# ArmingLou/seed-vc

Measured on AMD Instinct MI355X. Metric: mel_frames_per_sec, higher is better.
Workload: dtype f16; 1 GPU; seed-uvit-tat-xlsr-tiny CFM 25 steps cfg 0.7 + HiFT, batch 64 x (P=430,S=430) per GPU; batch_per_gpu=64, global_batch=64, prompt_frames=430, diffusion_steps=25, vocoder_precision=fp16p8, lanes_per_gpu=2, parallelism=utterance-sharded x1, audio gather on rank 0

## Files before the change

### seed-vc_amd/csrc/common.h

```cpp
#pragma once
#include <atomic>
#include <hip/hip_runtime.h>
#include <stdint.h>
#include <stdio.h>
#include <string>

namespace svc {

typedef _Float16 half_t;
typedef _Float16 half8 __attribute__((ext_vector_type(8)));
typedef _Float16 half4 __attribute__((ext_vector_type(4)));
typedef _Float16 half2v __attribute__((ext_vector_type(2)));
typedef float float4v __attribute__((ext_vector_type(4)));
typedef unsigned int u32x4 __attribute__((ext_vector_type(4)));

void set_error(const std::string& msg);
const char* get_error();

#define SVC_CHECK_HIP(expr)                                                                  \
    do {                                                                                     \
        hipError_t _e = (expr);                                                              \
        if (_e != hipSuccess) {                                                              \
            svc::set_error(std::string(#expr) + ": " + hipGetErrorString(_e) + " at " + __FILE__ + \
                           ":" + std::to_string(__LINE__));                                  \
            return 1;                                                                        \
        }                                                                                    \
    } while (0)

#define SVC_REQUIRE(cond, msg)                                                               \
    do {                                                                                     \
        if (!(cond)) {                                                                       \
            svc::set_error(std::string("requirement failed: ") + #cond + " -- " + (msg));    \
            return 1;                                                                        \
        }                                                                                    \
    } while (0)

__device__ __forceinline__ float sin_sq(float x) {
    const float n = rintf(x * 0.318309886183790672f);
    float r = fmaf(n, -3.140625f, x);
    r = fmaf(n, -9.67502593994140625e-4f, r);
    r = fmaf(n, -1.509957990978376e-7f, r);
    const float r2 = r * r;
    float p = fmaf(r2, 2.6348154733568663e-06f, -0.00019822761532850564f);
    p = fmaf(p, r2, 0.008333242498338223f);
    p = fmaf(p, r2, -0.1666666567325592f);
    const float sn = fmaf(p * r2, r, r);
    return sn * sn;
}

struct DeviceState {
    int device = -1;
    void* zero_page = nullptr;
    std::atomic<unsigned long long> kconv_attr{0};
    std::atomic<bool> fused_attr{false};
};
DeviceState* device_state();
int current_device();

enum { PROF_KGEMM_F16 = 0, PROF_KGEMM_F32 = 1, PROF_ATTN = 2, PROF_FUSED = 3, PROF_N = 4 };
bool prof_enabled();
void prof_begin(int cls, hipStream_t st);
void prof_end(int cls, double flops, double bytes, hipStream_t st, unsigned long long tag = 0);

template <int MAXA, int DPT>
__device__ __forceinline__ void wait_tiles(int ahead) {
    static_assert(MAXA * DPT <= 63, "vmcnt is a 6-bit counter");
    if constexpr (MAXA <= 0) {
        asm volatile("s_waitcnt vmcnt(0)" ::: "memory");
    } else {
        if (ahead >= MAXA) asm volatile("s_waitcnt vmcnt(%0)" ::"n"(MAXA * DPT) : "memory");
        else wait_tiles<MAXA - 1, DPT>(ahead);
    }
}

__device__ __forceinline__ float act_apply(float v, int act, float slope);
__device__ __forceinline__ uint4 pack8(const float* v) {
    half8 h;
#pragma unroll
    for (int j = 0; j < 8; ++j) h[j] = (half_t)v[j];
    return *reinterpret_cast<uint4*>(&h);
}

static inline int cdiv(long a, long b) { return (int)((a + b - 1) / b); }
static inline long round_up(long a, long b) { return (a + b - 1) / b * b; }

constexpr int KG_MAX_TAPS = 48;

enum { KG_PAD_ZERO = 0, KG_PAD_REFLECT = 1, KG_PAD_CLAMP = 2 };
enum { KG_ACT_NONE = 0, KG_ACT_SILU = 1, KG_ACT_ELU = 2, KG_ACT_LRELU = 3, KG_ACT_TANH = 4, KG_ACT_ABS = 5,
       KG_ACT_CLAMP = 6 , KG_ACT_SIGMOID = 7 };
enum {
    KG_EPI_STORE = 0,
    KG_EPI_SWIGLU = 1,
    KG_EPI_TANHSIG = 2,
    KG_EPI_QKV_ROPE = 3,
};

__device__ __forceinline__ float act_apply(float v, int act, float slope) {
    switch (act) {
        case KG_ACT_SILU: return v / (1.0f + __expf(-v));
        case KG_ACT_ELU: return v > 0.f ? v : (expm1f(v));
        case KG_ACT_LRELU: return v > 0.f ? v : v * slope;
        case KG_ACT_TANH: return tanhf(v);
        case KG_ACT_ABS: return fabsf(v);
        case KG_ACT_CLAMP: return fminf(fmaxf(v, -slope), slope);
        case KG_ACT_SIGMOID: return 1.0f / (1.0f + __expf(-v));
        default: return v;
// ... 44 lines not shown
    const void* w; long ldw;
    const float* bias;
    int B, Lin, Lout, N, cin_pad, k, dil, pad_left, nsub;
    int c_seq_rows, c_off;
    float* c32; long ldc32;
    half_t* c16; half_t* c16_lo; long ldc16;
    const float* post_a; const float* post_ib; int post_n;
    const float* res; long ldres;
    const float* res2; long ldres2;
    float out_scale;
    int act; float act_slope;
    const void* zero_page;
    int w8_exp;
    int c16_lo_fmt;
    const int* seq_len;
};
bool kconv_enabled();
int kconv_launch(const KConvParams& p, hipStream_t st);
__device__ __forceinline__ unsigned lo_pair_p8(float hi_as_float, float lo) {
    const float a = __builtin_amdgcn_fmed3f(hi_as_float, -448.f, 448.f), b = __builtin_amdgcn_fmed3f(lo * 2048.f, -448.f, 448.f);
    return (unsigned)__builtin_amdgcn_cvt_pk_fp8_f32(a, b, 0, false) & 0xffffu;
}
int kconv_pack_p8(const float* src, unsigned short* dst, int n0, int n1, int n2, long s0, long s1, long s2, long d0, long d1, long d2,
                  const float* scale, int* exp_out, hipStream_t st);

struct PanelParams {
    int M;
    int Lout, seq_rows, row_off;
    const half_t* wstream;
    int n_slots;
    float eps;
    int do_post;
    const half_t* ao;
    float* x;
    const float* gate_a; const float* gate_f;
    const float* g_ffn; const float* w_f; const float* b_f; int add_one;
    int I;
    half_t* c16;
    int do_skip;
    const half_t* skip_in; const float* bskip;
    int do_qkv;
    const float* g_attn; const float* w_a; const float* b_a;
    const float* rope; float q_scale;
    half_t* qk; half_t* vt; long vt_seq_stride; long vt_ld; int vt_mode;
    int do_final;
    const float* g_fin; const float* w_fin; const float* b_fin; half_t* n16;
};
bool fused_supported(int D, int I);
long fused_stream_halfs(int D, int I, bool post, bool skip, bool qkv);
long fused_pack_stream(half_t* dst, int D, int I, const float* wo, const float* w1, const float* w3, const float* w2,
                       const float* wskip, const float* wqkv, hipStream_t st);
int fused_panel_launch(const PanelParams& p, int D, bool gated, hipStream_t st);

struct AttnParams {
    const half_t* q; const half_t* k; long ld_qk;
    const half_t* vt; long vt_seq_stride; long vt_ld;
    half_t* out; long ld_out;
    int n_seq, H, seq_rows, Tq;
    int q_start;
    const int* kv_len; int kv_len_const;
    int vt_perm;
};
__host__ __device__ inline int vt_perm_pos(int pos) {
    return (pos & ~31) | (((pos >> 2) & 3) << 3) | (((pos >> 4) & 1) << 2) | (pos & 3);
}
__host__ __device__ inline int vt_perm_pos16(int pos) {
    return (pos & ~12) | ((pos & 4) << 1) | ((pos & 8) >> 1);
}
__host__ __device__ inline int vt_pos(int pos, int mode) {
    return mode == 2 ? vt_perm_pos16(pos) : (mode == 1 ? vt_perm_pos(pos) : pos);
}
int attention_vt_mode(int n_seq, int H, int Tq);
int attention_launch(const AttnParams& p, hipStream_t st);
int attention_permute_vt(half_t* vt, long rows, long vt_ld, int mode, hipStream_t st);

int rmsnorm_mod_launch(const float* x, long ldx, half_t* y, long ldy, const float* gamma,
                       const float* w, const float* b, long ld_wb, int add_one,
                       int rows, int D, int seq_rows, float eps, hipStream_t st);
int layernorm_mod_launch(const float* x, long ldx, half_t* y, long ldy, const float* scale,
                         const float* shift, int rows, int D, float eps, hipStream_t st);

}
```

### seed-vc_amd/csrc/dit.hip

```cpp
#include <math.h>
#include <string.h>

#include <algorithm>
#include <vector>

#include "model_util.h"

using namespace svc;

namespace {
constexpr int MAX_STREAMS = 3;
constexpr int ROPE_POS = 8192;

float bf16_round(float f) {
    uint32_t u;
    memcpy(&u, &f, 4);
    u = (u + 0x7FFF + ((u >> 16) & 1)) & 0xFFFF0000u;
    memcpy(&f, &u, 4);
    return f;
}

std::vector<float> linspace01(int n) {
    std::vector<float> v(n);
    const float step = 1.0f / (float)(n - 1);
    const int half = n / 2;
    for (int i = 0; i < n; ++i) v[i] = i < half ? 0.0f + step * (float)i : 1.0f - step * (float)(n - 1 - i);
    return v;
}
}

struct svc_dit {
    svc_dit_config_t cfg;
    int D, H, L, C, Dc, S, I, W, NL, WK, npre, C16, C32;
    bool v2, wavenet, adaptive_blocks;
    Arena wts, ws;
    struct StepGraph {
        std::vector<float> key;
        hipGraphExec_t exec = nullptr;
        int seen = 0;
    };
    std::vector<StepGraph> graphs;
    hipStream_t cap_stream = nullptr;
    int use_graphs = 0;
    void drop_graphs() {
        for (auto& g : graphs) if (g.exec) (void)hipGraphExecDestroy(g.exec);
        graphs.clear();
    }
    PinnedRing staging;
    hipStream_t create_stream;
    int device = -1;

    struct Layer {
        half_t *wqkv, *wo, *w13, *w2, *wskip;
        float *bskip, *g_attn, *g_ffn;
        half_t* stream = nullptr;
        int stream_slots = 0;
    };
    half_t* stream_pre = nullptr;
    int stream_pre_slots = 0;
    bool fused_ok = false;
    long fused_min_rows = 10240;
    std::vector<Layer> layers;
    float* g_final;
    std::vector<int> emit, recv;
    float *te_w0, *te_b0, *te_w2, *te_b2, *te_freqs;
    float *te2_w0, *te2_b0, *te2_w2, *te2_b2, *te2_freqs;
    float *mod_w, *mod_b;
    int mod_n;
    int mod_layer_n;
    half_t* w_merge_x;
    float* w_stat;
    float* stat_const;
    float* w_style_merge;
    float *style_in_w, *style_in_b;
    half_t *head_wa, *head_w2;
    float *head_b0, *head_b2;
    half_t *w_longskip, *w_conv1, *w_resproj, *w_fl, *w_conv2;
    float *b_longskip, *b_conv1, *b_resproj, *b_fl, *b_conv2;
    float *wn_cond_w, *wn_cond_b, *fl_mod_w, *fl_mod_b;
    std::vector<half_t*> wn_in, wn_res, wn_skip;
    std::vector<float*> wn_res_b, wn_skip_b;
    half_t* wn_tail = nullptr;
    float* b_tail = nullptr;
    long acts_stride = 0;
    float* rope;

    int cap_streams = 0, cap_B = 0, cap_T = 0, cap_steps = 0;
    int seq_rows = 0, vt_ld = 0;
    float *x32, *xin, *st_term, *v32, *u_rowvec, *tok_style, *prompt32, *wnx32, *flin32;
    half_t *x16, *n16, *qk16, *vt, *ao16, *ff16, *h16, *hm16, *xr16, *wnx16, *acts16, *fl16, *fo16;
    std::vector<half_t*> skip16;
    int *d_kvlen, *d_convlen, *d_plen;
    int* d_convlen_w = nullptr;
    int win0 = 0;
    float *d_tvals, *d_tfeat, *d_th, *d_t1, *d_t1s, *d_t2, *d_mod, *d_gcond, *d_flmod, *d_stylevec;
    int microbatch = 0;

    int pack(const StateDict& sd, hipStream_t st);
    int reserve(int n_streams, int B, int T, int n_steps, hipStream_t st);
    int tables(const std::vector<float>& tvals, hipStream_t st);
    int statics(int n_streams, const int (*flags)[3], int B, int T, const float* mu, const float* style_dev,
                hipStream_t st);
    int run_group(const svc_cfm_args_t* a, int b0, int nb, int n_streams, const int (*flags)[3],
                  const std::vector<float>& tvals, const std::vector<float>& dts, float c0, float ca, float cb,
                  int stream_a, int stream_b, hipStream_t st);
    int body(int n_streams, int B, int T, int step, hipStream_t st);
    int body_fused(int n_streams, int B, int T, int step, hipStream_t st);
    int head(int n_streams, int B, int T, int step, hipStream_t st);
};

namespace {

int pack_block(int dtype, const float* src, long src_ld, long src_col, int N, int K, void* dst, long ldw, long dst_col,
               long dst_row0, long dst_row_step, const float* scale, hipStream_t st) {
    return pack_any(dtype, src + src_col, dst, dst_row0 * ldw + dst_col, N, 1, K, src_ld, 0, 1, dst_row_step * ldw, 0, 1,
                    scale, st);
}

float* copy_vec(Arena& ar, const float* src, long n, hipStream_t st) {
    float* d = ar.alloc_n<float>(n, st);
    if (!d) return nullptr;
    if (hipMemcpyAsync(d, src, n * sizeof(float), hipMemcpyDeviceToDevice, st) != hipSuccess) {
        set_error("hipMemcpyAsync failed");
        return nullptr;
    }
    return d;
}

}

#define GETW(var, name, ...)                                              \
    const svc_tensor_desc_t* var = sd.get(name);                          \
    if (require_shape(var, name, {__VA_ARGS__})) return 1;

int svc_dit::pack(const StateDict& sd, hipStream_t st) {
    const long Dp = round_up(D, 128);
    auto new16 = [&](long rows, long ld) { return wts.alloc_n<half_t>(round_up(rows, 128) * ld, st); };
    layers.resize(L);
    for (int i = 0; i < L; ++i) {
        const std::string p = "transformer.layers." + std::to_string(i) + ".";
        Layer& ly = layers[i];
        GETW(wqkv, p + "attention.wqkv.weight", 3 * D, D);
        GETW(wo, p + "attention.wo.weight", D, D);
        GETW(w1, p + "feed_forward.w1.weight", I, D);
        GETW(w3, p + "feed_forward.w3.weight", I, D);
        GETW(w2, p + "feed_forward.w2.weight", D, I);
        ly.wqkv = new16(3 * D, D);
        ly.wo = new16(D, D);
        ly.w13 = new16(2 * I, D);
        ly.w2 = new16(D, I);
        if (!ly.wqkv || !ly.wo || !ly.w13 || !ly.w2) return 1;
        if (pack_block(0, wqkv->data, D, 0, 3 * D, D, ly.wqkv, D, 0, 0, 1, nullptr, st)) return 1;
        if (pack_block(0, wo->data, D, 0, D, D, ly.wo, D, 0, 0, 1, nullptr, st)) return 1;
        if (pack_block(0, w1->data, D, 0, I, D, ly.w13, D, 0, 0, 2, nullptr, st)) return 1;
        if (pack_block(0, w3->data, D, 0, I, D, ly.w13, D, 0, 1, 2, nullptr, st)) return 1;
        if (pack_block(0, w2->data, I, 0, D, I, ly.w2, I, 0, 0, 1, nullptr, st)) return 1;
        const std::string an = v2 ? p + "attention_norm.norm.weight" : p + "attention_norm.norm.weight";
        const std::string fn = v2 ? p + "ffn_norm.weight" : p + "ffn_norm.norm.weight";
        GETW(ga, an, D);
// ... 350 lines not shown
    d_gcond = ws.alloc_n<float>(Sx * std::max(2L * W * NL, 1L), st);
    d_flmod = ws.alloc_n<float>(Sx * std::max(2 * W, 1), st);
    d_stylevec = ws.alloc_n<float>((long)cap_B * D, st);
    if (!d_kvlen || !d_convlen || !d_convlen_w || !d_plen || !d_tvals || !d_tfeat || !d_th || !d_t1 || !d_t1s || !d_t2 || !d_mod ||
        !d_gcond || !d_flmod || !d_stylevec)
        return 1;
    seq_rows = (int)round_up(T + npre, 8);
    vt_ld = (int)round_up(seq_rows, 64);
    SVC_CHECK_HIP(hipStreamSynchronize(st));
    return 0;
}

int svc_dit::tables(const std::vector<float>& tvals, hipStream_t st) {
    const int n = (int)tvals.size();
    {
        float* h = reinterpret_cast<float*>(staging.acquire(n * sizeof(float)));
        if (!h) return 1;
        memcpy(h, tvals.data(), n * sizeof(float));
        SVC_CHECK_HIP(hipMemcpyAsync(d_tvals, h, n * sizeof(float), hipMemcpyHostToDevice, st));
        if (staging.commit(st)) return 1;
    }
    if (timestep_feat_launch(d_tvals, te_freqs, d_tfeat, n, st)) return 1;
    if (small_linear_launch(d_tfeat, 256, te_w0, 256, te_b0, d_th, D, n, D, 256, KG_ACT_SILU, st)) return 1;
    if (small_linear_launch(d_th, D, te_w2, D, te_b2, d_t1, D, n, D, D, KG_ACT_NONE, st)) return 1;
    if (silu_launch(d_t1, d_t1s, (long)n * D, st)) return 1;
    if (small_linear_launch(v2 ? d_t1s : d_t1, D, mod_w, D, mod_b, d_mod, mod_n, n, mod_n, D, KG_ACT_NONE, st)) return 1;
    if (wavenet) {
        if (small_linear_launch(d_tfeat, 256, te2_w0, 256, te2_b0, d_th, W, n, W, 256, KG_ACT_SILU, st)) return 1;
        if (small_linear_launch(d_th, W, te2_w2, W, te2_b2, d_t2, W, n, W, W, KG_ACT_NONE, st)) return 1;
        if (small_linear_launch(d_t2, W, wn_cond_w, W, wn_cond_b, d_gcond, 2L * W * NL, n, 2 * W * NL, W, KG_ACT_NONE, st)) return 1;
        if (small_linear_launch(d_t1s, D, fl_mod_w, W, fl_mod_b, d_flmod, 2 * W, n, 2 * W, W, KG_ACT_NONE, st)) return 1;
    }
    return 0;
}


namespace {
KGemmParams gemm_base(int M, int N, int Lout) {
    KGemmParams p;
    memset(&p, 0, sizeof(p));
    p.M = M;
    p.N = N;
    p.Lout = Lout;
    p.a_seq_rows = Lout;
    p.c_seq_rows = Lout;
    p.a_stride = 1;
    p.a_len = Lout;
    p.n_taps = 1;
    p.vec_ok = 1;
    return p;
}
}

int svc_dit::body(int n_streams, int B, int T, int step, hipStream_t st) {
    const int nseq = n_streams * B;
    const int M = nseq * seq_rows;
    const float* mod = d_mod + (long)step * mod_n;
    if (prefix_rows_launch(xin, nseq, seq_rows, D, npre, T + npre, d_t1 + (long)step * D, tok_style,
                           cfg.time_as_token ? 1 : 0, st)) return 1;
    {
        KGemmParams p = gemm_base(nseq * T, D, T);
        p.a_ptr[0] = x16; p.a_ld[0] = C16; p.a_ktiles[0] = C16 / 64;
        p.a_seq_rows = seq_rows; p.a_len = T;
        p.w = w_merge_x; p.ldw = C16;
        p.c_seq_rows = seq_rows; p.c_off = npre;
        p.c32 = xin; p.ldc32 = D;
        p.res = st_term; p.ldres = D;
        if (kgemm_launch(p, 0, KG_EPI_STORE, st)) return 1;
    }
    if (fused_ok && (long)M >= fused_min_rows) {
        if (body_fused(n_streams, B, T, step, st)) return 1;
        return head(n_streams, B, T, step, st);
    }
    const int Lw = seq_rows - win0;
    auto gemm_win = [&](int N) {
        KGemmParams p = gemm_base(nseq * Lw, N, Lw);
        p.a_seq_rows = seq_rows; p.c_seq_rows = seq_rows;
        p.a_off = win0; p.c_off = win0;
        return p;
    };
    size_t emit_i = 0;
    std::vector<int> skip_stack;
    for (int i = 0; i < L; ++i) {
        const bool tail_only = i == L - 1 && win0 > 0;

        const Layer& ly = layers[i];
        const float* lmod = adaptive_blocks ? mod + (long)i * mod_layer_n : nullptr;
        const bool is_recv = ly.wskip != nullptr;
        if (is_recv) {
            const int src = skip_stack.back();
            skip_stack.pop_back();
            KGemmParams p = gemm_base(M, D, seq_rows);
            p.n_taps = 2;
            p.a_ptr[0] = h16; p.a_ld[0] = D; p.a_ktiles[0] = D / 64;
            p.a_ptr[1] = skip16[src]; p.a_ld[1] = D; p.a_ktiles[1] = D / 64;
            p.w = ly.wskip; p.ldw = 2 * D;
            p.bias = ly.bskip;
            p.c32 = xin; p.ldc32 = D;
            if (kgemm_launch(p, 0, KG_EPI_STORE, st)) return 1;
        }
        const float *w_a = nullptr, *b_a = nullptr, *gate_a = nullptr, *w_f = nullptr, *b_f = nullptr, *gate_f = nullptr;
        if (lmod) {
            if (v2) {
                b_a = lmod; w_a = lmod + D; gate_a = lmod + 2 * D;
                b_f = lmod + 3 * D; w_f = lmod + 4 * D; gate_f = lmod + 5 * D;
            } else {
                w_a = lmod; b_a = lmod + D; w_f = lmod + 2 * D; b_f = lmod + 3 * D;
            }
        }
        if (rmsnorm_mod_launch(xin, D, n16, D, ly.g_attn, w_a, b_a, 0, v2 ? 1 : 0, M, D, seq_rows, 1e-5f, st)) return 1;
        {
            KGemmParams p = gemm_base(M, 3 * D, seq_rows);
            p.a_ptr[0] = n16; p.a_ld[0] = D; p.a_ktiles[0] = D / 64;
            p.w = ly.wqkv; p.ldw = D;
            p.c16 = qk16; p.ldc16 = 2 * D;
            p.rope = rope; p.rope_D = D; p.q_scale = 0.125f * 1.4426950408889634f;
            p.vt = vt; p.vt_seq_stride = (long)D * vt_ld; p.vt_ld = vt_ld; p.vt_mode = attention_vt_mode(nseq, H, seq_rows);
            if (kgemm_launch(p, 0, KG_EPI_QKV_ROPE, st)) return 1;
        }
        {
            AttnParams a;
            memset(&a, 0, sizeof(a));
            a.q = qk16; a.k = qk16 + D; a.ld_qk = 2 * D;
            a.vt = vt; a.vt_seq_stride = (long)D * vt_ld; a.vt_ld = vt_ld; a.vt_perm = attention_vt_mode(nseq, H, seq_rows);
            a.out = ao16; a.ld_out = D;
            a.n_seq = nseq; a.H = H; a.seq_rows = seq_rows; a.Tq = seq_rows;
            a.q_start = tail_only ? win0 : 0;
            a.kv_len = d_kvlen;
            if (attention_launch(a, st)) return 1;
        }
        {
            KGemmParams p = tail_only ? gemm_win(D) : gemm_base(M, D, seq_rows);
            p.a_ptr[0] = ao16; p.a_ld[0] = D; p.a_ktiles[0] = D / 64;
            p.w = ly.wo; p.ldw = D;
            p.gate = gate_a; p.ld_gate = 0;
            p.res = xin; p.ldres = D;
            p.c32 = xin; p.ldc32 = D;
            if (kgemm_launch(p, 0, KG_EPI_STORE, st)) return 1;
        }
        if (rmsnorm_mod_launch(xin, D, n16, D, ly.g_ffn, w_f, b_f, 0, v2 ? 1 : 0, M, D, seq_rows, 1e-5f, st)) return 1;
        {
            KGemmParams p = tail_only ? gemm_win(2 * I) : gemm_base(M, 2 * I, seq_rows);
            p.a_ptr[0] = n16; p.a_ld[0] = D; p.a_ktiles[0] = D / 64;
            p.w = ly.w13; p.ldw = D;
            p.c16 = ff16; p.ldc16 = I;
            if (kgemm_launch(p, 0, KG_EPI_SWIGLU, st)) return 1;
        }
        {
            KGemmParams p = tail_only ? gemm_win(D) : gemm_base(M, D, seq_rows);
            p.a_ptr[0] = ff16; p.a_ld[0] = I; p.a_ktiles[0] = I / 64;
            p.w = ly.w2; p.ldw = I;
            p.gate = gate_f; p.ld_gate = 0;
            p.res = xin; p.ldres = D;
            p.c32 = xin; p.ldc32 = D;
            const bool is_emit = std::find(emit.begin(), emit.end(), i) != emit.end();
            const bool next_recv = i + 1 < L && layers[i + 1].wskip != nullptr;
            if (is_emit) {
                p.c16 = skip16[emit_i]; p.ldc16 = D;
                skip_stack.push_back((int)emit_i);
                ++emit_i;
            } else if (next_recv) {
                p.c16 = h16; p.ldc16 = D;
            }
            if (kgemm_launch(p, 0, KG_EPI_STORE, st)) return 1;
        }
    }
    {
        const float* fm = mod + (long)L * mod_layer_n;
        const float* w = fm;
        const float* b = fm + D;
        if (rmsnorm_mod_launch(xin, D, n16, D, g_final, w, b, 0, v2 ? 1 : 0, M, D, seq_rows, 1e-5f, st)) return 1;
    }
    return head(n_streams, B, T, step, st);
}

int svc_dit::head(int n_streams, int B, int T, int step, hipStream_t st) {
    const int nseq = n_streams * B;
    const int M = nseq * seq_rows;
    const int Lw = seq_rows - win0;
    auto gemm_win = [&](int N) {
        KGemmParams p = gemm_base(nseq * Lw, N, Lw);
        p.a_seq_rows = seq_rows; p.c_seq_rows = seq_rows;
        p.a_off = win0; p.c_off = win0;
        return p;
    };
    if (!wavenet) {
        {
            KGemmParams p = gemm_win(D);
            p.a_ptr[0] = n16; p.a_ld[0] = D; p.a_ktiles[0] = D / 64;
            p.w = head_wa; p.ldw = D; p.bias = head_b0; p.act = KG_ACT_SILU;
            p.c16 = hm16; p.ldc16 = D;
            if (kgemm_launch(p, 0, KG_EPI_STORE, st)) return 1;
        }
        {
            KGemmParams p = gemm_win(C);
            p.a_ptr[0] = hm16; p.a_ld[0] = D; p.a_ktiles[0] = D / 64;
            p.w = head_w2; p.ldw = D; p.bias = head_b2;
            p.c32 = v32; p.ldc32 = C16;
            if (kgemm_launch(p, 0, KG_EPI_STORE, st)) return 1;
        }
        return 0;
    }
    const half_t* xres16 = n16;
    if (cfg.long_skip_connection) {
        KGemmParams p = gemm_win(D);
        p.n_taps = 2;
        p.a_ptr[0] = n16; p.a_ld[0] = D; p.a_ktiles[0] = D / 64;
        p.a_ptr[1] = x16; p.a_ld[1] = C16; p.a_ktiles[1] = C16 / 64;
        p.w = w_longskip; p.ldw = D + C16; p.bias = b_longskip;
        p.c16 = xr16; p.ldc16 = D;
        if (kgemm_launch(p, 0, KG_EPI_STORE, st)) return 1;
        xres16 = xr16;
    }
    {
        KGemmParams p = gemm_win(W);
        p.a_ptr[0] = xres16; p.a_ld[0] = D; p.a_ktiles[0] = D / 64;
        p.w = w_conv1; p.ldw = D; p.bias = b_conv1;
        p.c32 = wnx32; p.ldc32 = W; p.c16 = wnx16; p.ldc16 = W;
        if (kgemm_launch(p, 0, KG_EPI_STORE, st)) return 1;
    }
    for (int i = 0; i < NL; ++i) {
        int dil = 1;
        for (int j = 0; j < i; ++j) dil *= cfg.wn_dilation_rate;
        {
            KGemmParams p = gemm_win(2 * W);
            p.n_taps = WK;
// ... 174 lines not shown
    }
    return 0;
}

namespace {
__global__ void init_state_kernel(float* __restrict__ x, long ldx, half_t* __restrict__ x16, long ldx16, int rows, int B,
                                  int T, int C, const int* __restrict__ prompt_len, int n_copies, long copy_stride) {
    const long i = (long)blockIdx.x * blockDim.x + threadIdx.x;
    if (i >= (long)B * T * C) return;
    const int c = (int)(i % C);
    const long bt = i / C;
    const int t = (int)(bt % T), b = (int)(bt / T);
    const long o = ((long)b * rows + t) * ldx + c;
    float v = x[o];
    if (t < prompt_len[b]) v = 0.f;
    x[o] = v;
    for (int k = 0; k < n_copies; ++k) x16[k * copy_stride + ((long)b * rows + t) * ldx16 + c] = (half_t)v;
}

__global__ void euler_kernel(float* __restrict__ x, long ldx, half_t* __restrict__ x16, long ldx16, int rows,
                             const float* __restrict__ v, long ldv, long v_stream_stride, int v_off, int B, int T, int C,
                             const int* __restrict__ prompt_len, float dt, float c0, float ca, float cb, int stream_a,
                             int stream_b, int n_copies, long copy_stride) {
    const long i = (long)blockIdx.x * blockDim.x + threadIdx.x;
    if (i >= (long)B * T * C) return;
    const int c = (int)(i % C);
    const long bt = i / C;
    const int t = (int)(bt % T), b = (int)(bt / T);
    const long vo = ((long)b * rows + v_off + t) * ldv + c;
    float d = c0 * v[vo];
    if (stream_a >= 0) d -= ca * v[vo + stream_a * v_stream_stride];
    if (stream_b >= 0) d -= cb * v[vo + stream_b * v_stream_stride];
    const long xo = ((long)b * rows + t) * ldx + c;
    float nx = x[xo] + dt * d;
    if (t < prompt_len[b]) nx = 0.f;
    x[xo] = nx;
    for (int k = 0; k < n_copies; ++k) x16[k * copy_stride + ((long)b * rows + t) * ldx16 + c] = (half_t)nx;
}

__global__ void prompt_rows_kernel(const float* __restrict__ src, int C, int P, float* __restrict__ dst, long ld, int rows,
                                   int T, const int* __restrict__ prompt_len, int B) {
    const long i = (long)blockIdx.x * blockDim.x + threadIdx.x;
    if (i >= (long)B * T * C) return;
    const int t = (int)(i % T);
    const long bc = i / T;
    const int c = (int)(bc % C), b = (int)(bc / C);
    const float v = (t < prompt_len[b] && t < P) ? src[((long)b * C + c) * P + t] : 0.f;
    dst[((long)b * rows + t) * ld + c] = v;
}
}

int svc_dit::run_group(const svc_cfm_args_t* a, int b0, int nb, int n_streams, const int (*flags)[3],
                       const std::vector<float>& tvals, const std::vector<float>& dts, float c0, float ca, float cb,
                       int stream_a, int stream_b, hipStream_t st) {
    const int T = a->T, P = a->P;
    const int n_steps = (int)tvals.size();
    if (reserve(n_streams, nb, T, n_steps, st)) return 1;
    std::vector<int> kv(n_streams * nb), cv(n_streams * nb), pl(nb);
    for (int b = 0; b < nb; ++b) {
        const int len = a->x_lens ? (int)a->x_lens[b0 + b] : T;
        const int plen = a->prompt_lens ? (int)a->prompt_lens[b0 + b] : P;
        SVC_REQUIRE(len >= 1 && len <= T, "x_lens out of range");
        SVC_REQUIRE(plen >= 0 && plen <= P && plen <= len, "prompt_lens out of range");
        pl[b] = plen;
        for (int j = 0; j < n_streams; ++j) {
            kv[j * nb + b] = len + npre;
            cv[j * nb + b] = len;
        }
    }
    {
        int halo = 0;
        if (wavenet) {
            int dil = 1;
            for (int i = 0; i < NL; ++i) {
                const int total = (WK - 1) * dil;
                halo += total - total / 2;
                dil *= cfg.wn_dilation_rate;
            }
        }
        const int min_pl = *std::min_element(pl.begin(), pl.end());
        win0 = std::max(0, npre + min_pl - halo) & ~7;
    }
    std::vector<int> cvw(cv.size());
    for (size_t i = 0; i < cv.size(); ++i) cvw[i] = cv[i] - (win0 - npre > 0 ? win0 - npre : 0);
    {
        const size_t n = kv.size();
        int* h = reinterpret_cast<int*>(staging.acquire((3 * n + pl.size()) * sizeof(int)));
        if (!h) return 1;
        memcpy(h, kv.data(), n * 4); memcpy(h + n, cv.data(), n * 4); memcpy(h + 2 * n, cvw.data(), n * 4);
        memcpy(h + 3 * n, pl.data(), pl.size() * 4);
        SVC_CHECK_HIP(hipMemcpyAsync(d_kvlen, h, n * 4, hipMemcpyHostToDevice, st));
        SVC_CHECK_HIP(hipMemcpyAsync(d_convlen, h + n, n * 4, hipMemcpyHostToDevice, st));
        SVC_CHECK_HIP(hipMemcpyAsync(d_convlen_w, h + 2 * n, n * 4, hipMemcpyHostToDevice, st));
        SVC_CHECK_HIP(hipMemcpyAsync(d_plen, h + 3 * n, pl.size() * 4, hipMemcpyHostToDevice, st));
        if (staging.commit(st)) return 1;
    }
    if (tables(tvals, st)) return 1;

    const long copy_stride = (long)nb * seq_rows * C16;
    const long n_el = (long)nb * T * C;
    if (bct_to_btc_launch(a->z + (long)b0 * C * T, nb, C, T, x32, C16, nullptr, 0, seq_rows, T, a->temperature, st)) return 1;
    hipLaunchKernelGGL(init_state_kernel, dim3(cdiv(n_el, 256)), dim3(256), 0, st, x32, (long)C16, x16, (long)C16, seq_rows,
                       nb, T, C, d_plen, n_streams, copy_stride);
    SVC_CHECK_HIP(hipGetLastError());
    hipLaunchKernelGGL(prompt_rows_kernel, dim3(cdiv(n_el, 256)), dim3(256), 0, st, a->prompt + (long)b0 * C * P, C, P,
                       prompt32, (long)C32, seq_rows, T, d_plen, nb);
    SVC_CHECK_HIP(hipGetLastError());
    if (statics(n_streams, flags, nb, T, a->mu + (long)b0 * T * Dc, a->style + (long)b0 * S, st)) return 1;

    auto steps = [&](hipStream_t s_) -> int {
        for (int s = 0; s < n_steps; ++s) {
            if (body(n_streams, nb, T, s, s_)) return 1;
            hipLaunchKernelGGL(euler_kernel, dim3(cdiv(n_el, 256)), dim3(256), 0, s_, x32, (long)C16, x16, (long)C16, seq_rows,
                               v32, (long)C16, (long)nb * seq_rows * C16, npre, nb, T, C, d_plen, dts[s], c0, ca, cb,
                               stream_a, stream_b, n_streams, copy_stride);
            SVC_CHECK_HIP(hipGetLastError());
        }
        return 0;
    };
    static const int graph_env = [] { const char* e = getenv("SVC_DIT_GRAPH"); return e ? (e[0] == '0' ? 0 : 1) : -1; }();
    bool done = false;
    if ((graph_env >= 0 ? graph_env : use_graphs) && !prof_enabled()) {
        std::vector<float> key = {(float)n_streams, (float)nb, (float)T, (float)n_steps, (float)win0, (float)seq_rows, c0, ca, cb,
                                  (float)stream_a, (float)stream_b, (float)fused_min_rows};
        key.insert(key.end(), dts.begin(), dts.end());
        StepGraph* g = nullptr;
        for (auto& c : graphs) if (c.key == key) { g = &c; break; }
        if (!g) {
            if (graphs.size() >= 8) { if (graphs.front().exec) (void)hipGraphExecDestroy(graphs.front().exec); graphs.erase(graphs.begin()); }
            graphs.push_back(StepGraph());
            g = &graphs.back();
            g->key = key;
        }
        if (g->seen++ >= 1 && !g->exec) {
            if (!cap_stream && hipStreamCreateWithFlags(&cap_stream, hipStreamNonBlocking) != hipSuccess) { (void)hipGetLastError(); cap_stream = nullptr; }
            hipGraph_t gr = nullptr;
            if (cap_stream && hipStreamBeginCapture(cap_stream, hipStreamCaptureModeThreadLocal) == hipSuccess) {
                const int rc = steps(cap_stream);
                const hipError_t e = hipStreamEndCapture(cap_stream, &gr);
                if (rc == 0 && e == hipSuccess && gr && hipGraphInstantiate(&g->exec, gr, nullptr, nullptr, 0) != hipSuccess) g->exec = nullptr;
                if (gr) (void)hipGraphDestroy(gr);
                if (rc || e != hipSuccess) { (void)hipGetLastError(); g->exec = nullptr; if (rc) return 1; }
            } else {
                (void)hipGetLastError();
            }
        }
        if (g->exec) {
            SVC_CHECK_HIP(hipGraphLaunch(g->exec, st));
            done = true;
        }
    }
    if (!done && steps(st)) return 1;
    return btc_to_bct_launch(x32, C16, seq_rows, a->out + (long)b0 * C * T, nb, C, T, st);
}

extern "C" {

int svc_dit_create(const svc_dit_config_t* cfg, const svc_tensor_desc_t* weights, int n_weights, void* stream,
                   svc_dit_t** out) {
    SVC_REQUIRE(cfg && weights && out, "null argument");
    SVC_REQUIRE(cfg->hidden_dim == cfg->num_heads * 64, "head_dim must be 64 (hidden_dim = 64 * num_heads)");
    SVC_REQUIRE(cfg->content_dim % 32 == 0, "content_dim must be a multiple of 32");
    SVC_REQUIRE(cfg->in_channels % 8 == 0 && cfg->in_channels <= 128, "in_channels must be a multiple of 8, <= 128");
    svc_dit* m = new svc_dit();
    m->cfg = *cfg;
    m->device = current_device();
    m->v2 = cfg->version == 2;
    m->D = cfg->hidden_dim; m->H = cfg->num_heads; m->L = cfg->depth; m->C = cfg->in_channels;
    m->Dc = cfg->content_dim; m->S = cfg->style_dim;
    {
        const int n_hidden = (int)(2 * (4 * m->D) / 3);
        m->I = (int)round_up(n_hidden, 256);
    }
    m->wavenet = cfg->final_layer_type == 1;
    m->W = m->wavenet ? cfg->wn_hidden_dim : 0;
    m->NL = m->wavenet ? cfg->wn_num_layers : 0;
    m->WK = m->wavenet ? cfg->wn_kernel_size : 0;
// ... 49 lines not shown
int svc_dit_set_graphs(svc_dit_t* m, int on) {
    SVC_REQUIRE(m, "null argument");
    m->use_graphs = on ? 1 : 0;
    if (!on) m->drop_graphs();
    return 0;
}

int svc_cfm_sample(svc_dit_t* m, const svc_cfm_args_t* a, void* stream) {
    SVC_REQUIRE(m && a, "null argument");
    SVC_REQUIRE(a->B >= 1 && a->T >= 1 && a->P >= 0 && a->P <= a->T && a->n_timesteps >= 1, "bad sampler shape");
    SVC_REQUIRE(a->T + m->npre <= ROPE_POS, "sequence longer than the RoPE table");
    SVC_REQUIRE(a->mu && (a->prompt || a->P == 0) && a->style && a->z && a->out, "null tensor");
    SVC_REQUIRE(current_device() == m->device, "this handle was created on another device (make it current before the call)");
    hipStream_t st = (hipStream_t)stream;
    const int N = a->n_timesteps;
    std::vector<float> ts = linspace01(N + 1);
    std::vector<float> tvals(N), dts(N);
    if (!m->v2) {
        float t = ts[0];
        for (int s = 1; s <= N; ++s) {
            const float dt = ts[s] - ts[s - 1];
            tvals[s - 1] = t;
            dts[s - 1] = dt;
            t = t + dt;
        }
    } else {
        for (auto& v : ts) v = v + (-1.0f) * (cosf((float)M_PI / 2.0f * v) - 1.0f + v);
        float t = ts[0], dt = ts[1] - ts[0];
        for (int s = 1; s <= N; ++s) {
            tvals[s - 1] = t;
            dts[s - 1] = dt;
            t = t + dt;
            if (s < N) dt = ts[s + 1] - t;
        }
    }
    int flags[MAX_STREAMS][3] = {{1, 1, 1}, {0, 0, 0}, {0, 0, 0}};
    int n_streams = 1, sa = -1, sb = -1;
    float c0 = 1.f, ca = 0.f, cb = 0.f;
    const float ra = a->cfg_rate[0], rb = a->cfg_rate[1];
    if (!m->v2) {
        if (ra > 0.f) { n_streams = 2; sa = 1; c0 = 1.f + ra; ca = ra; }
    } else if (a->random_voice) {
        n_streams = 2; flags[0][0] = 0; flags[0][1] = 0; sa = 1; c0 = 1.f + ra; ca = ra;
    } else if (ra == 0.f && rb == 0.f) {
        n_streams = 1;
    } else if (ra == 0.f) {
        n_streams = 2; flags[1][2] = 1; sa = 1; c0 = 1.f + rb; ca = rb;
    } else if (rb == 0.f) {
        n_streams = 2; sa = 1; c0 = 1.f + ra; ca = ra;
    } else {
        n_streams = 3; flags[1][2] = 1; sa = 2; sb = 1; c0 = 1.f + ra + rb; ca = ra; cb = rb;
    }
    int mb = m->microbatch > 0 ? m->microbatch : 32;
    for (int b0 = 0; b0 < a->B; b0 += mb) {
        const int nb = std::min(mb, a->B - b0);
        if (m->run_group(a, b0, nb, n_streams, flags, tvals, dts, c0, ca, cb, sa, sb, st)) return 1;
    }
    return 0;
}

int svc_dit_forward(svc_dit_t* m, int N, int T, const float* x, const float* prompt_x, const int64_t* x_lens, float t,
                    const float* style, const float* mu, float* out, void* stream) {
    SVC_REQUIRE(m && x && prompt_x && style && mu && out, "null argument");
    SVC_REQUIRE(N >= 1 && T >= 1 && T + m->npre <= ROPE_POS, "bad estimator shape");
    SVC_REQUIRE(current_device() == m->device, "this handle was created on another device (make it current before the call)");
    hipStream_t st = (hipStream_t)stream;
    const int flags[1][3] = {{1, 1, 1}};
    if (m->reserve(1, N, T, 1, st)) return 1;
    std::vector<int> kv(N), cv(N), pl(N);
    for (int b = 0; b < N; ++b) {
        const int len = x_lens ? (int)x_lens[b] : T;
        SVC_REQUIRE(len >= 1 && len <= T, "x_lens out of range");
        kv[b] = len + m->npre; cv[b] = len; pl[b] = T;
    }
    m->win0 = 0;
    {
        int* h = reinterpret_cast<int*>(m->staging.acquire(3 * (size_t)N * sizeof(int)));
        if (!h) return 1;
        memcpy(h, kv.data(), N * 4); memcpy(h + N, cv.data(), N * 4); memcpy(h + 2 * N, pl.data(), N * 4);
        SVC_CHECK_HIP(hipMemcpyAsync(m->d_kvlen, h, N * 4, hipMemcpyHostToDevice, st));
        SVC_CHECK_HIP(hipMemcpyAsync(m->d_convlen, h + N, N * 4, hipMemcpyHostToDevice, st));
        SVC_CHECK_HIP(hipMemcpyAsync(m->d_convlen_w, h + N, N * 4, hipMemcpyHostToDevice, st));
        SVC_CHECK_HIP(hipMemcpyAsync(m->d_plen, h + 2 * N, N * 4, hipMemcpyHostToDevice, st));
        if (m->staging.commit(st)) return 1;
    }
    std::vector<float> tv(1, t);
    if (m->tables(tv, st)) return 1;
    const int C = m->C, C16 = m->C16, C32 = m->C32, rows = m->seq_rows;
    if (bct_to_btc_launch(x, N, C, T, m->x32, C16, m->x16, C16, rows, T, 1.0f, st)) return 1;
    const long n_el = (long)N * T * C;
    hipLaunchKernelGGL(prompt_rows_kernel, dim3(cdiv(n_el, 256)), dim3(256), 0, st, prompt_x, C, T, m->prompt32, (long)C32,
                       rows, T, m->d_plen, N);
    SVC_CHECK_HIP(hipGetLastError());
    if (m->statics(1, flags, N, T, mu, style, st)) return 1;
    if (m->body(1, N, T, 0, st)) return 1;
    return btc_to_bct_launch(m->v32 + (long)m->npre * C16, C16, rows, out, N, C, T, st);
}

}
```

Before: 135,800 mel-frames/s.

## Fuse CFM head, Euler update and next-step input merge into one seam kernel

Adds a seam kernel that runs the estimator head MLP for every guidance stream and combines the streams with the CFG coefficients. The same kernel applies the Euler update to the state and computes the next step's merged input rows, including prefix tokens. This replaces the separate head GEMMs, the euler kernel, the prefix-row kernel and the merge GEMM between DiT bodies. It removes several launches and round trips of intermediates through global memory. By default it is used only when the row count reaches a threshold, and the state is no longer replicated per stream.

```diff
diff --git a/seed-vc_amd/csrc/common.h b/seed-vc_amd/csrc/common.h
--- a/seed-vc_amd/csrc/common.h
+++ b/seed-vc_amd/csrc/common.h
@@ -53,6 +53,7 @@
     void* zero_page = nullptr;
     std::atomic<unsigned long long> kconv_attr{0};
     std::atomic<bool> fused_attr{false};
+    std::atomic<unsigned> seam_attr{0};
 };
 DeviceState* device_state();
 int current_device();
@@ -203,6 +204,27 @@
                        const float* wskip, const float* wqkv, hipStream_t st);
 int fused_panel_launch(const PanelParams& p, int D, bool gated, hipStream_t st);
 
+struct SeamParams {
+    int nb, n_streams, seq_rows, T, npre, win0, D, C, C16;
+    int do_head;
+    int do_merge;
+    const half_t* n16;
+    const half_t* head_wa; const half_t* head_w2;
+    const float* head_b0; const float* head_b2;
+    int n_comb; int order[3]; float coef[3];
+    float dt;
+    float* x32;
+    const int* prompt_len;
+    const half_t* w_merge_x;
+    const float* st_term;
+    float* xin;
+    const float* tok_time;
+    const float* tok_style;
+    int time_first;
+};
+bool cfm_seam_supported(int D, int C);
+int cfm_seam_launch(const SeamParams& p, hipStream_t st);
+
 struct AttnParams {
     const half_t* q; const half_t* k; long ld_qk;
     const half_t* vt; long vt_seq_stride; long vt_ld;
diff --git a/seed-vc_amd/csrc/dit.hip b/seed-vc_amd/csrc/dit.hip
--- a/seed-vc_amd/csrc/dit.hip
+++ b/seed-vc_amd/csrc/dit.hip
@@ -59,6 +59,7 @@
     half_t* stream_pre = nullptr;
     int stream_pre_slots = 0;
     bool fused_ok = false;
+    static constexpr long seam_min_rows = 49152;
     long fused_min_rows = 10240;
     std::vector<Layer> layers;
     float* g_final;
@@ -103,8 +104,10 @@
                 hipStream_t st);
     int run_group(const svc_cfm_args_t* a, int b0, int nb, int n_streams, const int (*flags)[3],
                   const std::vector<float>& tvals, const std::vector<float>& dts, float c0, float ca, float cb,
-                  int stream_a, int stream_b, hipStream_t st);
-    int body(int n_streams, int B, int T, int step, hipStream_t st);
+                  int stream_a, int stream_b, int seam_mode, hipStream_t st);
+    int body(int n_streams, int B, int T, int step, hipStream_t st, bool seam = false);
+    int seam(int n_streams, int B, int T, int step, int n_steps, bool do_head, float dt, float c0, float ca, float cb,
+             int stream_a, int stream_b, hipStream_t st);
     int body_fused(int n_streams, int B, int T, int step, hipStream_t st);
     int head(int n_streams, int B, int T, int step, hipStream_t st);
 };
@@ -561,13 +564,13 @@
 }
 }
 
-int svc_dit::body(int n_streams, int B, int T, int step, hipStream_t st) {
+int svc_dit::body(int n_streams, int B, int T, int step, hipStream_t st, bool seam) {
     const int nseq = n_streams * B;
     const int M = nseq * seq_rows;
     const float* mod = d_mod + (long)step * mod_n;
-    if (prefix_rows_launch(xin, nseq, seq_rows, D, npre, T + npre, d_t1 + (long)step * D, tok_style,
+    if (!seam && prefix_rows_launch(xin, nseq, seq_rows, D, npre, T + npre, d_t1 + (long)step * D, tok_style,
                            cfg.time_as_token ? 1 : 0, st)) return 1;
-    {
+    if (!seam) {
         KGemmParams p = gemm_base(nseq * T, D, T);
         p.a_ptr[0] = x16; p.a_ld[0] = C16; p.a_ktiles[0] = C16 / 64;
         p.a_seq_rows = seq_rows; p.a_len = T;
@@ -579,7 +582,7 @@
     }
     if (fused_ok && (long)M >= fused_min_rows) {
         if (body_fused(n_streams, B, T, step, st)) return 1;
-        return head(n_streams, B, T, step, st);
+        return seam ? 0 : head(n_streams, B, T, step, st);
     }
     const int Lw = seq_rows - win0;
     auto gemm_win = [&](int N) {
@@ -680,7 +683,28 @@
         const float* b = fm + D;
         if (rmsnorm_mod_launch(xin, D, n16, D, g_final, w, b, 0, v2 ? 1 : 0, M, D, seq_rows, 1e-5f, st)) return 1;
     }
-    return head(n_streams, B, T, step, st);
+    return seam ? 0 : head(n_streams, B, T, step, st);
+}
+
+int svc_dit::seam(int n_streams, int B, int T, int step, int n_steps, bool do_head, float dt, float c0, float ca, float cb,
+                  int stream_a, int stream_b, hipStream_t st) {
+    SeamParams p;
+    memset(&p, 0, sizeof(p));
+    p.nb = B; p.n_streams = n_streams; p.seq_rows = seq_rows; p.T = T; p.npre = npre; p.win0 = win0;
+    p.D = D; p.C = C; p.C16 = C16;
+    p.do_head = do_head ? 1 : 0;
+    const int next = do_head ? step + 1 : step;
+    p.do_merge = next < n_steps ? 1 : 0;
+    p.n16 = n16; p.head_wa = head_wa; p.head_w2 = head_w2; p.head_b0 = head_b0; p.head_b2 = head_b2;
+    p.n_comb = 1; p.order[0] = 0; p.coef[0] = c0;
+    if (stream_a >= 0) { p.order[p.n_comb] = stream_a; p.coef[p.n_comb] = ca; ++p.n_comb; }
+    if (stream_b >= 0) { p.order[p.n_comb] = stream_b; p.coef[p.n_comb] = cb; ++p.n_comb; }
+    p.dt = dt;
+    p.x32 = x32; p.prompt_len = d_plen;
+    p.w_merge_x = w_merge_x; p.st_term = st_term; p.xin = xin;
+    p.tok_time = d_t1 + (long)(p.do_merge ? next : 0) * D; p.tok_style = tok_style;
+    p.time_first = cfg.time_as_token ? 1 : 0;
+    return cfm_seam_launch(p, st);
 }
 
 int svc_dit::head(int n_streams, int B, int T, int step, hipStream_t st) {
@@ -961,7 +985,7 @@
 
 int svc_dit::run_group(const svc_cfm_args_t* a, int b0, int nb, int n_streams, const int (*flags)[3],
                        const std::vector<float>& tvals, const std::vector<float>& dts, float c0, float ca, float cb,
-                       int stream_a, int stream_b, hipStream_t st) {
+                       int stream_a, int stream_b, int seam_mode, hipStream_t st) {
     const int T = a->T, P = a->P;
     const int n_steps = (int)tvals.size();
     if (reserve(n_streams, nb, T, n_steps, st)) return 1;
@@ -1006,11 +1030,13 @@
     }
     if (tables(tvals, st)) return 1;
 
+    const bool use_seam = seam_mode != 0 && !wavenet && cfm_seam_supported(D, C) &&
+                          (seam_mode == 1 || (long)n_streams * nb * seq_rows >= seam_min_rows);
     const long copy_stride = (long)nb * seq_rows * C16;
     const long n_el = (long)nb * T * C;
     if (bct_to_btc_launch(a->z + (long)b0 * C * T, nb, C, T, x32, C16, nullptr, 0, seq_rows, T, a->temperature, st)) return 1;
     hipLaunchKernelGGL(init_state_kernel, dim3(cdiv(n_el, 256)), dim3(256), 0, st, x32, (long)C16, x16, (long)C16, seq_rows,
-                       nb, T, C, d_plen, n_streams, copy_stride);
+                       nb, T, C, d_plen, use_seam ? 0 : n_streams, copy_stride);
     SVC_CHECK_HIP(hipGetLastError());
     hipLaunchKernelGGL(prompt_rows_kernel, dim3(cdiv(n_el, 256)), dim3(256), 0, st, a->prompt + (long)b0 * C * P, C, P,
                        prompt32, (long)C32, seq_rows, T, d_plen, nb);
@@ -1019,6 +1045,12 @@
 
     auto steps = [&](hipStream_t s_) -> int {
         for (int s = 0; s < n_steps; ++s) {
+            if (use_seam) {
+                if (s == 0 && seam(n_streams, nb, T, 0, n_steps, false, 0.f, c0, ca, cb, stream_a, stream_b, s_)) return 1;
+                if (body(n_streams, nb, T, s, s_, true)) return 1;
+                if (seam(n_streams, nb, T, s, n_steps, true, dts[s], c0, ca, cb, stream_a, stream_b, s_)) return 1;
+                continue;
+            }
             if (body(n_streams, nb, T, s, s_)) return 1;
             hipLaunchKernelGGL(euler_kernel, dim3(cdiv(n_el, 256)), dim3(256), 0, s_, x32, (long)C16, x16, (long)C16, seq_rows,
                                v32, (long)C16, (long)nb * seq_rows * C16, npre, nb, T, C, d_plen, dts[s], c0, ca, cb,
@@ -1031,7 +1063,7 @@
     bool done = false;
     if ((graph_env >= 0 ? graph_env : use_graphs) && !prof_enabled()) {
         std::vector<float> key = {(float)n_streams, (float)nb, (float)T, (float)n_steps, (float)win0, (float)seq_rows, c0, ca, cb,
-                                  (float)stream_a, (float)stream_b, (float)fused_min_rows};
+                                  (float)stream_a, (float)stream_b, (float)fused_min_rows, use_seam ? 1.f : 0.f};
         key.insert(key.end(), dts.begin(), dts.end());
         StepGraph* g = nullptr;
         for (auto& c : graphs) if (c.key == key) { g = &c; break; }
@@ -1187,9 +1219,11 @@
         n_streams = 3; flags[1][2] = 1; sa = 2; sb = 1; c0 = 1.f + ra + rb; ca = ra; cb = rb;
     }
     int mb = m->microbatch > 0 ? m->microbatch : 32;
+    const char* seam_env = getenv("SVC_CFM_SEAM");
+    const int seam_mode = !seam_env ? 2 : (seam_env[0] == '0' ? 0 : 1);
     for (int b0 = 0; b0 < a->B; b0 += mb) {
         const int nb = std::min(mb, a->B - b0);
-        if (m->run_group(a, b0, nb, n_streams, flags, tvals, dts, c0, ca, cb, sa, sb, st)) return 1;
+        if (m->run_group(a, b0, nb, n_streams, flags, tvals, dts, c0, ca, cb, sa, sb, seam_mode, st)) return 1;
     }
     return 0;
 }
diff --git a/seed-vc_amd/csrc/seam.hip b/seed-vc_amd/csrc/seam.hip
--- /dev/null
+++ b/seed-vc_amd/csrc/seam.hip
@@ -0,0 +1,289 @@
+#include "common.h"
+
+namespace svc {
+
+namespace {
+
+#define MFMA(a, b, c) __builtin_amdgcn_mfma_f32_16x16x32_f16((a), (b), (c), 0, 0, 0)
+
+template <int KC>
+struct SG {
+    static constexpr int D = 32 * KC, NT = D / 16;
+    static constexpr int HF = 2 * KC + 8;
+    static constexpr int SF = HF > 32 ? HF : 32;
+    static constexpr int NLD = SF / 4;
+    static constexpr int SLAB = SF * 1024;
+    static constexpr int LDS = 2 * SLAB;
+    static_assert(SF % 4 == 0 && KC % 2 == 0, "slab geometry");
+};
+
+template <int KC>
+__global__ __launch_bounds__(256) void cfm_seam_kernel(const SeamParams p) {
+    using G = SG<KC>;
+    constexpr int D = G::D, NT = G::NT, NLD = G::NLD, SLAB = G::SLAB;
+    extern __shared__ __attribute__((aligned(16))) char smem[];
+
+    const int tid = threadIdx.x, lane = tid & 63;
+    const int wave = __builtin_amdgcn_readfirstlane(tid >> 6);
+    const int fr = lane & 15, fq = lane >> 4;
+    const int b = blockIdx.y;
+    const int n_win = (p.seq_rows - p.win0 + 63) / 64;
+
+    auto prefix_val = [&](int pos, long seq, int col) -> float4v {
+        const float* s = (p.time_first && pos == 0) ? p.tok_time : p.tok_style + seq * D;
+        return *reinterpret_cast<const float4v*>(s + col);
+    };
+
+    if ((int)blockIdx.x >= n_win) {
+        if (!p.do_merge) return;
+        const int r0 = ((int)blockIdx.x - n_win) * 64;
+        const int nrows = min(64, p.win0 - r0);
+        constexpr int NV = D / 4;
+        for (int j = 0; j < p.n_streams; ++j) {
+            const long seq = (long)j * p.nb + b;
+            for (int idx = tid; idx < nrows * NV; idx += 256) {
+                const int r = idx / NV, col = (idx - r * NV) * 4;
+                const int pos = r0 + r;
+                const long o = (seq * p.seq_rows + pos) * D + col;
+                float4v v = {0.f, 0.f, 0.f, 0.f};
+                if (pos < p.npre) v = prefix_val(pos, seq, col);
+                else if (pos - p.npre < p.T) v = *reinterpret_cast<const float4v*>(p.st_term + o);
+                *reinterpret_cast<float4v*>(p.xin + o) = v;
+            }
+        }
+        return;
+    }
+
+    const int pos = p.win0 + (int)blockIdx.x * 64 + wave * 16 + fr;
+    const bool rok = pos < p.seq_rows;
+    const int posc = rok ? pos : p.seq_rows - 1;
+    const int t = pos - p.npre;
+    const bool frame = rok && t >= 0 && t < p.T;
+    const int kc3n = (p.C + 31) / 32;
+    const int nt2 = 2 * kc3n;
+    const int pr = 8 * (fr >> 2) + (fr & 3);
+
+    const int nH = p.do_head ? p.n_comb * KC : 0;
+    const int nM = p.do_merge ? (NT + 7) / 8 : 0;
+    const int total = nH + nM;
+    if (total == 0) return;
+
+    uint4 stg[NLD];
+    auto issue = [&](int q) {
+#pragma unroll
+        for (int i = 0; i < NLD; ++i) {
+            const int f = 4 * i + wave;
+            uint4 v = {0u, 0u, 0u, 0u};
+            if (q < nH) {
+                const int nc = q % KC;
+                if (f < 2 * KC) {
+                    const int tl = f < KC ? 0 : 1, kc = f - tl * KC;
+                    v = *reinterpret_cast<const uint4*>(p.head_wa + (long)(32 * nc + pr + 4 * tl) * D + 32 * kc + 8 * fq);
+                } else if (f - 2 * KC < nt2) {
+                    const int t2 = f - 2 * KC;
+                    v = *reinterpret_cast<const uint4*>(p.head_w2 + (long)(32 * (t2 >> 1) + pr + 4 * (t2 & 1)) * D + 32 * nc + 8 * fq);
+                }
+            } else {
+                const int tile = 8 * (q - nH) + (f >> 2), k3 = f & 3;
+                if (f < 32 && tile < NT && k3 < kc3n)
+                    v = *reinterpret_cast<const uint4*>(p.w_merge_x + (long)(16 * tile + fr) * p.C16 + 32 * k3 + 8 * fq);
+            }
+            stg[i] = v;
+        }
+    };
+    auto commit = [&](char* buf) {
+#pragma unroll
+        for (int i = 0; i < NLD; ++i) *reinterpret_cast<uint4*>(buf + (4 * i + wave) * 1024 + lane * 16) = stg[i];
+    };
+    int q = 0, cur = 0;
+    issue(0);
+    commit(smem);
+    __syncthreads();
+    auto next = [&]() { if (q + 1 < total) issue(q + 1); };
+    auto flip = [&]() {
+        if (q + 1 < total) commit(smem + (cur ^ 1) * SLAB);
+        __syncthreads();
+        cur ^= 1;
+        ++q;
+    };
+#define FRAG(base, idx) (*reinterpret_cast<const half8*>((base) + (idx) * 1024))
+
+    float4v dacc[8];
+#pragma unroll
+    for (int t2 = 0; t2 < 8; ++t2) dacc[t2] = (float4v){0.f, 0.f, 0.f, 0.f};
+    if (p.do_head) {
+#pragma unroll 1
+        for (int i = 0; i < p.n_comb; ++i) {
+            const int j = p.order[i];
+            const half_t* arow = p.n16 + (((long)j * p.nb + b) * p.seq_rows + posc) * D + 8 * fq;
+            half8 bop[KC];
+#pragma unroll
+            for (int kc = 0; kc < KC; ++kc) bop[kc] = *reinterpret_cast<const half8*>(arow + 32 * kc);
+            float4v acc2[8];
+#pragma unroll
+            for (int t2 = 0; t2 < 8; ++t2) acc2[t2] = (float4v){0.f, 0.f, 0.f, 0.f};
+#pragma unroll 1
+            for (int nc = 0; nc < KC; ++nc) {
+                next();
+                const char* base = smem + cur * SLAB + lane * 16;
+                float4v a0 = {0.f, 0.f, 0.f, 0.f}, a1 = a0;
+#pragma unroll
+                for (int kc = 0; kc < KC; ++kc) {
+                    a0 = MFMA(FRAG(base, kc), bop[kc], a0);
+                    a1 = MFMA(FRAG(base, KC + kc), bop[kc], a1);
+                }
+                const float4v b00 = *reinterpret_cast<const float4v*>(p.head_b0 + 32 * nc + 8 * fq);
+                const float4v b01 = *reinterpret_cast<const float4v*>(p.head_b0 + 32 * nc + 8 * fq + 4);
+                half8 hq;
+#pragma unroll
+                for (int r = 0; r < 4; ++r) {
+                    hq[r] = (half_t)act_apply(a0[r] + b00[r], KG_ACT_SILU, 0.f);
+                    hq[4 + r] = (half_t)act_apply(a1[r] + b01[r], KG_ACT_SILU, 0.f);
+                }
+#pragma unroll
+                for (int t2 = 0; t2 < 8; ++t2)
+                    if (t2 < nt2) acc2[t2] = MFMA(FRAG(base, 2 * KC + t2), hq, acc2[t2]);
+                flip();
+            }
+            const float cf = p.coef[i];
+#pragma unroll
+            for (int t2 = 0; t2 < 8; ++t2) {
+                const int col = 32 * (t2 >> 1) + 8 * fq + 4 * (t2 & 1);
+                if (t2 < nt2 && col < p.C) {
+                    const float4v b2 = *reinterpret_cast<const float4v*>(p.head_b2 + col);
+#pragma unroll
+                    for (int r = 0; r < 4; ++r) {
+                        const float v = acc2[t2][r] + b2[r];
+                        if (i == 0) dacc[t2][r] = cf * v;
+                        else dacc[t2][r] -= cf * v;
+                    }
+                }
+            }
+        }
+    }
+
+    half8 xb[4];
+    {
+        const int plen = p.prompt_len[b];
+        float4v nx[8];
+#pragma unroll
+        for (int t2 = 0; t2 < 8; ++t2) {
+            nx[t2] = (float4v){0.f, 0.f, 0.f, 0.f};
+            const int col = 32 * (t2 >> 1) + 8 * fq + 4 * (t2 & 1);
+            if (t2 < nt2 && col < p.C && frame) {
+                float* xp = p.x32 + ((long)b * p.seq_rows + t) * p.C16 + col;
+                const float4v x = *reinterpret_cast<const float4v*>(xp);
+                if (p.do_head) {
+#pragma unroll
+                    for (int r = 0; r < 4; ++r) {
+                        float v = x[r] + p.dt * dacc[t2][r];
+                        if (t < plen) v = 0.f;
+                        nx[t2][r] = v;
+                    }
+                    *reinterpret_cast<float4v*>(xp) = nx[t2];
+                } else {
+                    nx[t2] = x;
+                }
+            }
+        }
+#pragma unroll
+        for (int k3 = 0; k3 < 4; ++k3)
+#pragma unroll
+            for (int r = 0; r < 4; ++r) {
+                xb[k3][r] = (half_t)nx[2 * k3][r];
+                xb[k3][4 + r] = (half_t)nx[2 * k3 + 1][r];
+            }
+    }
+
+    if (p.do_merge) {
+#pragma unroll 1
+        for (int s3 = 0; s3 < nM; ++s3) {
+            next();
+            const char* base = smem + cur * SLAB + lane * 16;
+            float4v acc3[8];
+#pragma unroll
+            for (int t8 = 0; t8 < 8; ++t8) acc3[t8] = (float4v){0.f, 0.f, 0.f, 0.f};
+#pragma unroll
+            for (int k3 = 0; k3 < 4; ++k3)
+                if (k3 < kc3n) {
+#pragma unroll
+                    for (int t8 = 0; t8 < 8; ++t8) acc3[t8] = MFMA(FRAG(base, 4 * t8 + k3), xb[k3], acc3[t8]);
+                }
+            if (rok) {
+                for (int j = 0; j < p.n_streams; ++j) {
+                    const long seq = (long)j * p.nb + b;
+                    const long o = (seq * p.seq_rows + pos) * D + 4 * fq;
+#pragma unroll
+                    for (int t8 = 0; t8 < 8; ++t8) {
+                        const int tile = 8 * s3 + t8;
+                        if (tile < NT) {
+                            float4v v = {0.f, 0.f, 0.f, 0.f};
+                            if (frame) v = acc3[t8] + *reinterpret_cast<const float4v*>(p.st_term + o + 16 * tile);
+                            else if (pos < p.npre) v = prefix_val(pos, seq, 16 * tile + 4 * fq);
+                            *reinterpret_cast<float4v*>(p.xin + o + 16 * tile) = v;
+                        }
+                    }
+                }
+            }
+            flip();
+        }
+    }
+#undef FRAG
+}
+
+template <int KC>
+int launch(const SeamParams& p, unsigned bit, hipStream_t st) {
+    using G = SG<KC>;
+    DeviceState* ds = device_state();
+    if (!ds) return 1;
+    if (!(ds->seam_attr.load() & bit)) {
+        SVC_CHECK_HIP(hipFuncSetAttribute(reinterpret_cast<const void*>(&cfm_seam_kernel<KC>),
+                                          hipFuncAttributeMaxDynamicSharedMemorySize, G::LDS));
+        ds->seam_attr.fetch_or(bit);
+    }
+    const int n_win = cdiv(p.seq_rows - p.win0, 64), n_copy = p.do_merge ? cdiv(p.win0, 64) : 0;
+    if (n_win + n_copy == 0) return 0;
+    hipLaunchKernelGGL(cfm_seam_kernel<KC>, dim3(n_win + n_copy, p.nb), dim3(256), G::LDS, st, p);
+    SVC_CHECK_HIP(hipGetLastError());
+    return 0;
+}
+
+}
+
+bool cfm_seam_supported(int D, int C) {
+    return (D == 128 || D == 192 || D == 384 || D == 512) && C % 8 == 0 && C >= 8 && C <= 128;
+}
+
+int cfm_seam_launch(const SeamParams& p, hipStream_t st) {
+    SVC_REQUIRE(cfm_seam_supported(p.D, p.C), "seam kernel: unsupported width");
+    SVC_REQUIRE(p.nb >= 1 && p.n_streams >= 1 && p.win0 >= 0 && p.win0 <= p.seq_rows && p.win0 % 8 == 0, "seam kernel: bad geometry");
+    SVC_REQUIRE(p.do_head || p.do_merge, "seam kernel: nothing to do");
+    SVC_REQUIRE(!p.do_head || (p.n_comb >= 1 && p.n_comb <= 3), "seam kernel: guidance streams");
+    const bool prof = prof_enabled();
+    if (prof) prof_begin(PROF_KGEMM_F16, st);
+    int rc = 1;
+    switch (p.D) {
+        case 128: rc = launch<4>(p, 1u, st); break;
+        case 192: rc = launch<6>(p, 2u, st); break;
+        case 384: rc = launch<12>(p, 4u, st); break;
+        case 512: rc = launch<16>(p, 8u, st); break;
+    }
+    if (prof) {
+        const double rw = (double)p.nb * (p.seq_rows - p.win0), ra = (double)p.nb * p.seq_rows;
+        double flops = 0, bytes = 0;
+        if (p.do_head) {
+            flops += 2.0 * rw * p.n_comb * ((double)p.D * p.D + (double)p.D * p.C);
+            bytes += rw * p.n_comb * p.D * 2.0 + rw * p.C * 8.0 + ((double)p.D * p.D + (double)p.D * p.C) * 2.0;
+        }
+        if (p.do_merge) {
+            flops += 2.0 * rw * p.D * p.C;
+            bytes += ra * p.n_streams * p.D * 8.0 + (double)p.D * p.C * 2.0 + (p.do_head ? 0.0 : rw * p.C * 4.0);
+        }
+        const unsigned long long tag = ((unsigned long long)(long)rw << 40) | ((unsigned long long)(p.D & 0xFFFFF) << 20) |
+                                       ((unsigned long long)(p.C & 0xFFFF) << 4) | 0xFu;
+        prof_end(PROF_KGEMM_F16, flops, bytes, st, tag);
+    }
+    return rc;
+}
+
+}
```

After: 136,200 mel-frames/s, median of 6. Within noise of the previous version (+0.3%).
